# Wangkkkkkkkk/ORB-SLAM3

Measured on AMD Instinct MI355X. Metric: ORB extract+match frames/sec @752x480, 1000 feat, higher is better.
Workload: dtype u8; 1 GPU; configs[1]: 752x480 grayscale (synthetic, texture class 'dense', 16 distinct frames per rank), 1000 features, 8 levels, scale 1.2, FAST 20/7; batch of 1024 frames/GPU/step resident in HBM; extract + AssignFeaturesToGrid + SearchByProjection(frame, previous frame, th=15, mono; ORBmatcher.cc:2469-2711) of every frame, final match rows (claims, TH_HIGH, rotation-histogram cull) on the device; keypoin; launch=hipGraph replay (one hipGraphLaunch per step), keypoints_last_batch=1035840

## Files before the change

orb-slam3_amd/csrc/orbm_api.hip:

```cpp
#include "../../include/orbm.h"
#include "orbm_kernels.hip.h"

#include <cstdarg>
#include <cstdio>
#include <algorithm>
#include <chrono>
#include <climits>
#include <cmath>
#include <cstring>
#include <string>
#include <utility>
#include <vector>

using namespace orbmk;

#ifdef ORBX_AB
static inline const char* ab_env(const char* name) { return getenv(name); }
#else
static inline const char* ab_env(const char*) { return nullptr; }
#endif

static thread_local std::string g_merr;
static void set_merr(const char* fmt, ...) {
    char buf[512];
// ... 960 lines not shown
    int nFused = 0;
    for (int i = 0; i < nq; ++i) {
        best_idx[i] = -1;
        if (!valid[i] || cnt[i] == 0) continue;
        int bestDist = chi2_gate ? 256 : INT_MAX, bestIdx = -1;
        for (int c = 0; c < cnt[i]; ++c) {
            const int k = idx[(size_t)i * cap + c];
            if (chi2_gate) {
                const orbm_kp_t& kp = kf->kps[k];
                if (kf->uright && kf->uright[k] >= 0) {
                    const float ex = u[i] - kp.x, ey = v[i] - kp.y, er = ur[i] - kf->uright[k];
                    const float e2 = ex * ex + ey * ey + er * er;
                    if (e2 * inv_sigma2[kp.octave] > 7.8) continue;
                } else {
                    const float ex = u[i] - kp.x, ey = v[i] - kp.y;
                    const float e2 = ex * ex + ey * ey;
                    if (e2 * inv_sigma2[kp.octave] > 5.99) continue;
                }
            }
            const int d = dist[(size_t)i * cap + c];
            if (d < bestDist) { bestDist = d; bestIdx = k; }
        }
        if (bestDist <= ORBM_TH_LOW) { best_idx[i] = bestIdx; nFused++; }
    }
    return nFused;
}

static int sim3_one_way(orbm* m, const orbm_frame_t* src, const orbm_frame_t* dst, const float* sf_dst, const uint8_t* valid,
                        const float* u, const float* v, const int32_t* level, const uint8_t* qdesc, float th, std::vector<int>& vnMatch) {
    const int nq = src->n;
    vnMatch.assign(nq, -1);
    std::vector<float> qr(nq);
    std::vector<int> minl(nq), maxl(nq);
    for (int i = 0; i < nq; ++i) {
        if (!valid[i]) { qr[i] = -1.f; minl[i] = 0; maxl[i] = -1; continue; }
        qr[i] = th * sf_dst[level[i]]; minl[i] = level[i] - 1; maxl[i] = level[i];
    }
    int cap = std::max(1, std::min(dst->n, 2048));
    std::vector<int> cnt, idx, dist;
    orbm_frame_t f = *dst; f.uright = nullptr;
    int rc = window_pass(m, &f, nq, u, v, qr.data(), minl.data(), maxl.data(), nullptr, nullptr, qdesc, cap, cnt, idx, dist);
    if (rc) return rc;
    for (int i = 0; i < nq; ++i) {
        if (!valid[i]) continue;
        int bestDist = INT_MAX, bestIdx = -1;
        for (int c = 0; c < cnt[i]; ++c) {
            const int d = dist[(size_t)i * cap + c];
            if (d < bestDist) { bestDist = d; bestIdx = idx[(size_t)i * cap + c]; }
        }
        if (bestDist <= ORBM_TH_HIGH) vnMatch[i] = bestIdx;
    }
    return ORBM_OK;
}

int orbm_search_by_sim3(orbm_t* m, const orbm_frame_t* kf1, const orbm_frame_t* kf2, const float* sf1, const float* sf2,
                        const uint8_t* valid1, const float* u1, const float* v1, const int32_t* level1, const uint8_t* qdesc1,
                        const uint8_t* valid2, const float* u2, const float* v2, const int32_t* level2, const uint8_t* qdesc2,
                        float th, int32_t* matches12) {
    if (!m || !kf1 || !kf2) return ORBM_E_INVALID;
    std::vector<int> vnMatch1, vnMatch2;
    int rc = sim3_one_way(m, kf1, kf2, sf2, valid1, u1, v1, level1, qdesc1, th, vnMatch1);
    if (rc) return rc;
    rc = sim3_one_way(m, kf2, kf1, sf1, valid2, u2, v2, level2, qdesc2, th, vnMatch2);
    if (rc) return rc;
    int nFound = 0;
    for (int i1 = 0; i1 < kf1->n; ++i1) {
        matches12[i1] = -1;
        const int idx2 = vnMatch1[i1];
        if (idx2 >= 0 && vnMatch2[idx2] == i1) { matches12[i1] = idx2; nFound++; }
    }
    return nFound;
}

int orbm_grid_build_batch_async(orbm_t* m, const orbm_kp_t* kps, const int32_t* counts, int nframes, int cap,
                                float min_x, float min_y, float inv_w, float inv_h, int32_t* grid_start, int32_t* grid_idx) {
    if (!m || !kps || !counts || !grid_start || !grid_idx || nframes < 1 || cap < 1 || cap > 65535) return ORBM_E_INVALID;
    MHIPCHK(hipSetDevice(m->device));
    int n2 = 64; while (n2 < cap) n2 <<= 1;
    if ((size_t)n2 * 4 > 150 * 1024) { set_merr("too many keypoints per frame for the LDS sort"); return ORBM_E_CAPACITY; }
    if (cap > GRID_CS_MAX && n2 * 4 > 48 * 1024) MHIPCHK(hipFuncSetAttribute((const void*)k_grid_build_batch, hipFuncAttributeMaxDynamicSharedMemorySize, n2 * 4));
    MHIPCHK(rec_time(m, m->e2));
    m->gridFirst = true;
    if (cap <= GRID_CS_MAX)
        hipLaunchKernelGGL(k_grid_build_batch_cs, dim3(nframes), dim3(256), grid_cs_lds(cap), m->stream, (const KpIn*)kps, counts, cap,
                           min_x, min_y, inv_w, inv_h, grid_start, grid_idx);
    else
        hipLaunchKernelGGL(k_grid_build_batch, dim3(nframes), dim3(256), (size_t)n2 * 4, m->stream, (const KpIn*)kps, counts, cap, n2,
                           min_x, min_y, inv_w, inv_h, grid_start, grid_idx);
    MHIPCHK(hipGetLastError());
    return ORBM_OK;
}

static ScaleTab scale_tab(const float* sf, int nlevels) {
    ScaleTab st;
    for (int i = 0; i < 12; ++i) st.sf[i] = i < nlevels ? sf[i] : sf[nlevels - 1];
    return st;
}

static int lp_capacity(const char* call, int cap, int q_stride, int nlevels, int nbatch, const char* batch_name) {
    if (cap > 65535) { set_merr("%s: %d keypoint slots per frame (the candidate words hold 65535)", call, cap); return ORBM_E_CAPACITY; }
    if (q_stride > ORBM_LP_MAX_QUERIES) { set_merr("%s: q_stride %d above %d", call, q_stride, (int)ORBM_LP_MAX_QUERIES); return ORBM_E_CAPACITY; }
    if (nlevels > 12) { set_merr("%s: %d scale levels (the scale table holds 12)", call, nlevels); return ORBM_E_CAPACITY; }
    if (nbatch > 65535) { set_merr("%s: %d %s in one call (at most 65535)", call, nbatch, batch_name); return ORBM_E_CAPACITY; }
    return ORBM_OK;
}

int orbm_track_window_batch_async(orbm_t* m, const orbm_kp_t* kps, const uint8_t* desc, const int32_t* counts, int cap,
                                  const int32_t* grid_start, const int32_t* grid_idx,
                                  float min_x, float min_y, float inv_w, float inv_h,
                                  int q_first, int t_first, int npairs, float th, const float* sf, int nlevels,
                                  float dx, float dy, int32_t* best_idx, int32_t* best_dist, int32_t* second_dist) {
    if (!m || !kps || !desc || !counts || !grid_start || !grid_idx || !best_idx || !best_dist || !second_dist || npairs < 1 ||
        nlevels < 1 || nlevels > 12 || !sf) return ORBM_E_INVALID;
    MHIPCHK(hipSetDevice(m->device));
    const ScaleTab st = scale_tab(sf, nlevels);
    MHIPCHK(rec_time(m, m->e0));
    hipLaunchKernelGGL(k_track_window, dim3((cap + 3) / 4, npairs), dim3(256), 0, m->stream, (const KpIn*)kps, desc, counts, cap,
                       grid_start, grid_idx, min_x, min_y, inv_w, inv_h, q_first, t_first, th, st, dx, dy, best_idx, best_dist, second_dist);
    MHIPCHK(rec_time(m, m->e1));
    MHIPCHK(hipGetLastError());
    m->timed = true;
    return ORBM_OK;
}

int orbm_search_by_projection_batch_async(orbm_t* m, const orbm_kp_t* kps, const uint8_t* desc, const int32_t* counts, int cap,
                                          const int32_t* grid_start, const int32_t* grid_idx,
                                          float min_x, float min_y, float inv_w, float inv_h,
                                          int q_first, int t_first, int npairs, float th, const float* sf, int nlevels,
                                          float dx, float dy, const uint8_t* t_blocked, const uint8_t* q_obs, int check_orientation,
                                          int32_t* match, int32_t* nmatches) {
    if (!m || !kps || !desc || !counts || !grid_start || !grid_idx || !match || !nmatches || npairs < 1 || cap < 1 || cap > 65535 ||
        nlevels < 1 || nlevels > 12 || !sf || q_first < 0 || t_first < 0) return ORBM_E_INVALID;
    MHIPCHK(hipSetDevice(m->device));
    const ScaleTab st = scale_tab(sf, nlevels);
    const size_t lds = (size_t)(2 * ((cap + 31) >> 5) + 32 + cap) * sizeof(unsigned);
    if (lds > 64 * 1024) { set_merr("SearchByProjection batch: %d keypoint slots per frame need %zu B of LDS (limit 64 KB, ~16 000 slots)", cap, lds); return ORBM_E_INVALID; }
    const size_t rows = (size_t)npairs * cap;
    const size_t bCnt = (rows * sizeof(int) + 255) & ~(size_t)255, bKeys = (rows * TK_K * sizeof(unsigned) + 255) & ~(size_t)255,
                 bAcc = (rows * sizeof(unsigned) + 255) & ~(size_t)255, bEnt = rows * sizeof(uint4);
    uint8_t* scr = batch_scratch(m, bCnt + bKeys + bAcc + bEnt);
    if (!scr) { set_merr("SearchByProjection batch scratch of %zu B unavailable (inside a capture, run the call once eagerly first)", bCnt + bKeys + bAcc + bEnt); return ORBM_E_HIP; }
    int* topCnt = (int*)scr; unsigned* topKeys = (unsigned*)(scr + bCnt); unsigned* acc = (unsigned*)(scr + bCnt + bKeys);
    uint4* ent = (uint4*)(scr + bCnt + bKeys + bAcc);
    const float factor = ORBM_HISTO_LENGTH / 360.0f;
    MHIPCHK(rec_time(m, m->e0));
#ifdef ORBX_AB
    if (ab_env("ORBM_TOPK_WAVE"))
        hipLaunchKernelGGL(k_track_topk, dim3((cap + 3) / 4, npairs), dim3(256), 0, m->stream, (const KpIn*)kps, desc, counts, cap,
                           grid_start, grid_idx, min_x, min_y, inv_w, inv_h, q_first, t_first, th, st, dx, dy, factor, topCnt, topKeys);
    else
#endif
    {
        hipLaunchKernelGGL(k_track_pack, dim3((cap + 255) / 256, npairs), dim3(256), 0, m->stream, (const KpIn*)kps, cap, grid_start, grid_idx, t_first, ent);
        hipLaunchKernelGGL(k_track_topk16, dim3((cap + 15) / 16, npairs), dim3(256), 0, m->stream, (const KpIn*)kps, desc, counts, cap,
                           grid_start, ent, min_x, min_y, inv_w, inv_h, q_first, t_first, th, st, dx, dy, factor, topCnt, topKeys);
    }
#ifdef ORBX_AB
    if (ab_env("ORBM_CLAIM_V1"))
        hipLaunchKernelGGL(k_track_claim, dim3(npairs), dim3(64), lds, m->stream, (const KpIn*)kps, desc, counts, cap,
                           grid_start, grid_idx, min_x, min_y, inv_w, inv_h, q_first, t_first, th, st, dx, dy, factor, topCnt, topKeys,
                           t_blocked, q_obs, check_orientation, acc, match, nmatches);
    else
#endif
    hipLaunchKernelGGL(k_track_claim64, dim3(npairs), dim3(64), lds, m->stream, (const KpIn*)kps, desc, counts, cap,
                       grid_start, grid_idx, min_x, min_y, inv_w, inv_h, q_first, t_first, th, st, dx, dy, factor, topCnt, topKeys,
                       t_blocked, q_obs, check_orientation, acc, match, nmatches);
    MHIPCHK(rec_time(m, m->e1));
    MHIPCHK(hipGetLastError());
    m->timed = true;
    return ORBM_OK;
}

int orbm_search_by_projection_points_batch_async(orbm_t* m, const orbm_kp_t* kps, const uint8_t* desc, const int32_t* counts, int cap,
                                                 const int32_t* grid_start, const int32_t* grid_idx,
                                                 float min_x, float min_y, float inv_w, float inv_h, int t_first, int nframes,
                                                 const float* uright, const uint8_t* t_blocked, const int32_t* nq, int q_stride,
                                                 const uint8_t* in_view, const float* proj_x, const float* proj_y, const float* proj_xr,
                                                 const float* view_cos, const int32_t* level, const float* depth, float th_far,
                                                 const uint8_t* qdesc, const uint8_t* mp_obs, int q_shared,
                                                 float th, float nnratio, const float* scale_factors_host, int nlevels,
                                                 int32_t* match, int32_t* nmatches) {
    if (!m || !kps || !desc || !counts || !grid_start || !grid_idx || !nq || !in_view || !proj_x || !proj_y || !view_cos || !level ||
        !qdesc || !mp_obs || !match || !nmatches || !scale_factors_host || (uright && !proj_xr)) {
        set_merr("SearchByProjection points batch: a required array is NULL (proj_xr is required with uright)");
        return ORBM_E_INVALID;
    }
    if (nframes < 1 || cap < 1 || q_stride < 1 || t_first < 0 || nlevels < 1) {
        set_merr("SearchByProjection points batch: nframes, cap, q_stride and nlevels must be >= 1, t_first >= 0");
        return ORBM_E_INVALID;
    }
    if (const int rc = lp_capacity("SearchByProjection points batch", cap, q_stride, nlevels, nframes, "frames")) return rc;
    MHIPCHK(hipSetDevice(m->device));
    const ScaleTab st = scale_tab(scale_factors_host, nlevels);
    const size_t lds = (size_t)(((cap + 31) >> 5) + 32 + 64 * TK_K) * sizeof(unsigned);
    const size_t rows = (size_t)nframes * q_stride;
    const size_t bCnt = (rows * sizeof(int) + 255) & ~(size_t)255, bKeys = rows * TK_K * sizeof(unsigned), bR = rows * sizeof(float);
    uint8_t* scr = batch_scratch(m, bCnt + bKeys + bR);
    if (!scr) { set_merr("SearchByProjection points batch scratch of %zu B unavailable (inside a capture, run the call once eagerly first)", bCnt + bKeys + bR); return ORBM_E_HIP; }
    int* topCnt = (int*)scr; unsigned* topKeys = (unsigned*)(scr + bCnt); float* topR = (float*)(scr + bCnt + bKeys);
    LpRows R;
    R.nq = nq; R.q_stride = q_stride;
    R.in_view = in_view; R.px = proj_x; R.py = proj_y; R.pxr = proj_xr; R.view_cos = view_cos; R.level = level;
    R.depth = depth; R.th_far = th_far;
    R.qdesc = qdesc; R.mp_obs = mp_obs; R.q_shared = q_shared != 0;
    R.th = th; R.nlevels = nlevels;
    MHIPCHK(rec_time(m, m->e0));
    hipLaunchKernelGGL(k_lp_topk, dim3((q_stride + 3) / 4, nframes), dim3(256), 0, m->stream, (const KpIn*)kps, desc, cap, grid_start, grid_idx,
                       min_x, min_y, inv_w, inv_h, t_first, uright, R, st, topCnt, topKeys, topR);
    hipLaunchKernelGGL(k_lp_claim, dim3(nframes), dim3(64), lds, m->stream, (const KpIn*)kps, desc, counts, cap, grid_start, grid_idx,
                       min_x, min_y, inv_w, inv_h, t_first, uright, t_blocked, R, nnratio, topCnt, topKeys, topR, match, nmatches);
    MHIPCHK(rec_time(m, m->e1));
    MHIPCHK(hipGetLastError());
    m->timed = true;
    return ORBM_OK;
}

int orbm_search_by_projection_frame_batch_async(orbm_t* m, const orbm_kp_t* kps, const uint8_t* desc, const int32_t* counts, int cap,
                                                const int32_t* grid_start, const int32_t* grid_idx,
                                                float min_x, float min_y, float inv_w, float inv_h, int t_first, int npairs,
                                                const float* uright, float mbf, const uint8_t* t_blocked, const uint8_t* dir,
                                                const int32_t* nq, int q_stride, const uint8_t* valid, const float* u, const float* v,
                                                const float* invzc, const int32_t* octave, const float* angle, const uint8_t* qdesc,
                                                const uint8_t* mp_obs, float th, int retry_below, const float* scale_factors_host, int nlevels,
                                                int check_orientation, int32_t* match, int32_t* nmatches, uint8_t* retried) {
    if (!m || !kps || !desc || !counts || !grid_start || !grid_idx || !nq || !valid || !u || !v || !octave || !angle || !qdesc || !mp_obs ||
        !match || !nmatches || !scale_factors_host || (uright && !invzc)) {
        set_merr("SearchByProjection frame batch: a required array is NULL (invzc is required with uright)");
        return ORBM_E_INVALID;
    }
    if (npairs < 1 || cap < 1 || q_stride < 1 || t_first < 0 || nlevels < 1 || retry_below < 0) {
        set_merr("SearchByProjection frame batch: npairs, cap, q_stride and nlevels must be >= 1, t_first and retry_below >= 0");
        return ORBM_E_INVALID;
    }
    if (const int rc = lp_capacity("SearchByProjection frame batch", cap, q_stride, nlevels, npairs, "pairs")) return rc;
    MHIPCHK(hipSetDevice(m->device));
    const ScaleTab st = scale_tab(scale_factors_host, nlevels);
    const size_t lds = (size_t)(((cap + 31) >> 5) + 32 + 64 * TK_K) * sizeof(unsigned);
    const size_t rows = (size_t)npairs * q_stride;
    const size_t bCnt = (rows * sizeof(int) + 255) & ~(size_t)255, bKeys = rows * TK_K * sizeof(unsigned), bAcc = rows * sizeof(unsigned),
                 bR = rows * sizeof(float);
    uint8_t* scr = batch_scratch(m, bCnt + bKeys + bAcc + bR);
    if (!scr) { set_merr("SearchByProjection frame batch scratch of %zu B unavailable (inside a capture, run the call once eagerly first)", bCnt + bKeys + bAcc + bR); return ORBM_E_HIP; }
    int* topCnt = (int*)scr; unsigned* topKeys = (unsigned*)(scr + bCnt); unsigned* acc = (unsigned*)(scr + bCnt + bKeys);
    float* topR = (float*)(scr + bCnt + bKeys + bAcc);
    MmRows R;
    R.nq = nq; R.q_stride = q_stride;
    R.valid = valid; R.u = u; R.v = v; R.invzc = invzc; R.octave = octave; R.angle = angle;
    R.qdesc = qdesc; R.mp_obs = mp_obs; R.dir = dir;
    R.mbf = mbf; R.factor = ORBM_HISTO_LENGTH / 360.0f;
    R.nlevels = nlevels; R.retry_below = retry_below; R.check_ori = check_orientation != 0;
    const dim3 gTop((q_stride + 3) / 4, npairs);
    MHIPCHK(rec_time(m, m->e0));
    hipLaunchKernelGGL(k_mm_topk<false>, gTop, dim3(256), 0, m->stream, (const KpIn*)kps, desc, cap, grid_start, grid_idx,
                       min_x, min_y, inv_w, inv_h, t_first, uright, R, st, th, nmatches, topCnt, topKeys, topR);
    hipLaunchKernelGGL(k_mm_claim<false>, dim3(npairs), dim3(64), lds, m->stream, (const KpIn*)kps, desc, counts, cap, grid_start, grid_idx,
                       min_x, min_y, inv_w, inv_h, t_first, uright, t_blocked, R, topCnt, topKeys, topR, acc, match, nmatches, retried);
    if (retry_below > 0) {
        const float th2 = 2 * th;
        hipLaunchKernelGGL(k_mm_topk<true>, gTop, dim3(256), 0, m->stream, (const KpIn*)kps, desc, cap, grid_start, grid_idx,
                           min_x, min_y, inv_w, inv_h, t_first, uright, R, st, th2, nmatches, topCnt, topKeys, topR);
        hipLaunchKernelGGL(k_mm_claim<true>, dim3(npairs), dim3(64), lds, m->stream, (const KpIn*)kps, desc, counts, cap, grid_start, grid_idx,
                           min_x, min_y, inv_w, inv_h, t_first, uright, nullptr, R, topCnt, topKeys, topR, acc, match, nmatches, retried);
    }
    MHIPCHK(rec_time(m, m->e1));
    MHIPCHK(hipGetLastError());
    m->timed = true;
    return ORBM_OK;
}

int orbm_project_last_frame_batch_async(orbm_t* m, int npairs, const float* tcw_cur, const float* tcw_last, const int32_t* nq, int q_stride,
                                        const float* x3dw, const uint8_t* has_mp, const float* k_host, const float* bounds_host, float mb, int mono,
                                        uint8_t* valid, float* u, float* v, float* invzc, uint8_t* dir) {
    if (!m || !tcw_cur || !tcw_last || !nq || !x3dw || !has_mp || !k_host || !bounds_host || !valid || !u || !v || !invzc || !dir) {
        set_merr("project last frame batch: a required array is NULL");
        return ORBM_E_INVALID;
    }
    if (npairs < 1 || q_stride < 1) { set_merr("project last frame batch: npairs and q_stride must be >= 1"); return ORBM_E_INVALID; }
    if (q_stride > ORBM_LP_MAX_QUERIES) { set_merr("project last frame batch: q_stride %d above %d", q_stride, (int)ORBM_LP_MAX_QUERIES); return ORBM_E_CAPACITY; }
    if (npairs > 65535) { set_merr("project last frame batch: %d pairs in one call (at most 65535)", npairs); return ORBM_E_CAPACITY; }
    MHIPCHK(hipSetDevice(m->device));
    MmProj P;
    for (int i = 0; i < 4; ++i) { P.k[i] = k_host[i]; P.bounds[i] = bounds_host[i]; }
    P.mb = mb; P.mono = mono != 0; P.q_stride = q_stride;
    hipLaunchKernelGGL(k_mm_project, dim3((q_stride + 255) / 256, npairs), dim3(256), 0, m->stream, tcw_cur, tcw_last, nq, x3dw, has_mp, P,
                       valid, u, v, invzc, dir);
    MHIPCHK(hipGetLastError());
    return ORBM_OK;
}

int orbm_fuse_batch_async(orbm_t* m, int npairs,
                          int nkf_rows, int cap, const orbm_kp_t* kps_kf, const uint8_t* desc_kf, const float* uright_kf,
                          const int32_t* grid_start, const int32_t* grid_idx, float min_x, float min_y, float inv_w, float inv_h,
                          const int32_t* kf_row, const float* tcw, const float* ow,
                          const int32_t* nq, int q_stride, const uint8_t* valid,
                          const float* pw, const float* normal, const float* min_dist, const float* max_dist, const uint8_t* qdesc, int q_shared,
                          const float* k_host, const float* bounds_host, float bf,
                          float th, int chi2_gate, const float* scale_factors_host, const float* inv_sigma2_host,
                          float log_scale_factor, int nlevels,
                          int32_t* best_idx, int32_t* nfused, int32_t* level_out) {
    if (!m || !kps_kf || !desc_kf || !grid_start || !grid_idx || !tcw || !ow || !nq || !valid || !pw || !normal || !min_dist || !max_dist ||
        !qdesc || !k_host || !bounds_host || !scale_factors_host || (chi2_gate && !inv_sigma2_host) || !best_idx || !nfused) {
        set_merr("Fuse batch: a required array is NULL (inv_sigma2 is required with chi2_gate)");
        return ORBM_E_INVALID;
    }
    if (npairs < 1 || nkf_rows < 1 || cap < 1 || q_stride < 1 || nlevels < 1 || !std::isfinite(th)) {
        set_merr("Fuse batch: npairs, nkf_rows, cap, q_stride and nlevels must be >= 1, th finite");
// ... 913 lines not shown
```

orb-slam3_amd/csrc/orbm_kernels.hip.h:

```cpp
#pragma once
#include <hip/hip_runtime.h>
#include <stdint.h>

namespace orbmk {

typedef unsigned long long u64;

__device__ __forceinline__ int ham256(const u64 a[4], u64 b0, u64 b1, u64 b2, u64 b3) {
    return __popcll(a[0] ^ b0) + __popcll(a[1] ^ b1) + __popcll(a[2] ^ b2) + __popcll(a[3] ^ b3);
}

__device__ __forceinline__ unsigned bcnt_acc(unsigned x, unsigned acc) {
#if __HIP_DEVICE_COMPILE__
    unsigned r;
    asm("v_bcnt_u32_b32 %0, %1, %2" : "=v"(r) : "v"(x), "v"(acc));
    return r;
#else
    return (unsigned)__builtin_popcount(x) + acc;
#endif
}

__device__ __forceinline__ unsigned umed3(unsigned a, unsigned b, unsigned c) {
#if __HIP_DEVICE_COMPILE__
    unsigned r;
// ... 1106 lines not shown
        if (sz > max1) { max3 = max2; max2 = max1; max1 = sz; i3 = i2; i2 = i1; i1 = i; }
        else if (sz > max2) { max3 = max2; max2 = sz; i3 = i2; i2 = i; }
        else if (sz > max3) { max3 = sz; i3 = i; }
    }
    if ((float)max2 < 0.1f * (float)max1) { i2 = -1; i3 = -1; }
    else if ((float)max3 < 0.1f * (float)max1) i3 = -1;
    return Max3{i1, i2, i3};
}

__device__ __forceinline__ int rot_cull(const unsigned int* hist, const unsigned int* acc, int nacc, int* mrow, int lane) {
    const Max3 m3 = three_maxima(hist);
    const int i1 = m3.i1, i2 = m3.i2, i3 = m3.i3;
    int pruned = 0;
    for (int e = lane; e < nacc; e += 64) {
        const unsigned int v = acc[e];
        const int bin = (int)(v >> 16), k = (int)(v & 0xFFFFu);
        if (bin != i1 && bin != i2 && bin != i3) { mrow[k] = -2; ++pruned; }
    }
#pragma unroll
    for (int o = 32; o > 0; o >>= 1) pruned += __shfl_xor(pruned, o);
    return pruned;
}

__device__ __forceinline__ void put_topk(int* out_cnt, float* out_r, unsigned int* out_keys, size_t o, int cnt, float r, const u64 (&top)[TK_K]) {
    out_cnt[o] = cnt;
    out_r[o] = r;
    uint4* ok = (uint4*)(out_keys + o * TK_K);
    ok[0] = make_uint4(cand_word(top[0]), cand_word(top[1]), cand_word(top[2]), cand_word(top[3]));
    ok[1] = make_uint4(cand_word(top[4]), cand_word(top[5]), cand_word(top[6]), cand_word(top[7]));
}

#ifdef ORBX_AB
__global__ __launch_bounds__(256) void k_track_topk(const KpIn* __restrict__ kps, const uint8_t* __restrict__ desc,
                                                    const int* __restrict__ counts, int cap, const int* __restrict__ grid_start,
                                                    const int* __restrict__ grid_idx, float min_x, float min_y, float inv_w, float inv_h,
                                                    int q_first, int t_first, float th, ScaleTab st, float dx, float dy, float factor,
                                                    int* __restrict__ out_cnt, unsigned int* __restrict__ out_keys) {
    const int lane = threadIdx.x & 63;
    const int pair = blockIdx.y;
    const int qf = q_first + pair, tf = t_first + pair;
    const int q = blockIdx.x * 4 + (threadIdx.x >> 6);
    if (q >= min(counts[qf], cap)) return;
    const KpIn kq = kps[(size_t)qf * cap + q];
    const KpIn* kt = kps + (size_t)tf * cap;
    const uint8_t* dt = desc + (size_t)tf * cap * 32;
    const int* gs = grid_start + (size_t)tf * (64 * 48 + 1);
    const int* gi = grid_idx + (size_t)tf * cap;
    const float x = kq.x + dx, y = kq.y + dy, r = th * st.sf[kq.octave];
    const int minLevel = kq.octave - 1, maxLevel = kq.octave + 1;
    const unsigned INV = 0xFFFFFFFFu;
    unsigned topKey[TK_K], topPay[TK_K];
#pragma unroll
    for (int i = 0; i < TK_K; ++i) { topKey[i] = INV; topPay[i] = INV; }
    int cnt = 0;
    const int nMinCellX = max(0, (int)floorf((x - min_x - r) * inv_w));
    const int nMaxCellX = min(63, (int)ceilf((x - min_x + r) * inv_w));
    const int nMinCellY = max(0, (int)floorf((y - min_y - r) * inv_h));
    const int nMaxCellY = min(47, (int)ceilf((y - min_y + r) * inv_h));
    if (nMinCellX < 64 && nMaxCellX >= 0 && nMinCellY < 48 && nMaxCellY >= 0) {
        const uint4* qp = (const uint4*)(desc + ((size_t)qf * cap + q) * 32);
        const uint4 qlo = qp[0], qhi = qp[1];
        const u64 a[4] = {(u64)qlo.x | ((u64)qlo.y << 32), (u64)qlo.z | ((u64)qlo.w << 32),
                          (u64)qhi.x | ((u64)qhi.y << 32), (u64)qhi.z | ((u64)qhi.w << 32)};
        const unsigned long long lt = (1ull << lane) - 1ull;
        const int ncols = nMaxCellX - nMinCellX + 1;
        int cj0 = 0, clen = 0;
        if (lane < ncols) {
            const int ix = nMinCellX + lane;
            cj0 = gs[ix * 48 + nMinCellY];
            clen = gs[ix * 48 + nMaxCellY + 1] - cj0;
        }
        int total;
        const int coff = wave_excl_scan(clen, &total);
        bool first = true;
        for (int base = 0; base < total; base += 64) {
            const int t = base + lane;
            int myj0 = 0, myoff = 0;
            for (int c = 0; c < ncols; ++c) {
                const int oc = __builtin_amdgcn_readlane(coff, c), jc = __builtin_amdgcn_readlane(cj0, c);
                if (t >= oc) { myoff = oc; myj0 = jc; }
            }
            bool ok = false;
            int k = 0;
            float ang = 0.f;
            if (t < total) {
                k = gi[myj0 + (t - myoff)];
                const KpIn kp = kt[k];
                ok = !(kp.octave < minLevel) && !(kp.octave > maxLevel);
                if (!(fabsf(kp.x - x) < r && fabsf(kp.y - y) < r)) ok = false;
                ang = kp.angle;
            }
            const unsigned long long bal = __ballot(ok);
            if (bal == 0) continue;
            unsigned key = INV, pay = INV;
            if (ok) {
                const int pos = cnt + __popcll(bal & lt);
                const uint4* tp = (const uint4*)(dt + (size_t)k * 32);
                const uint4 lo = tp[0], hi = tp[1];
                const int d = ham256(a, (u64)lo.x | ((u64)lo.y << 32), (u64)lo.z | ((u64)lo.w << 32),
                                     (u64)hi.x | ((u64)hi.y << 32), (u64)hi.z | ((u64)hi.w << 32));
                float rot = kq.angle - ang;
                if (rot < 0.0f) rot += 360.0f;
                int bin = (int)roundf(rot * factor);
                if (bin == 30) bin = 0;
                if (bin < 0 || bin >= 30) bin = TK_NOBIN;
                key = ((unsigned)d << 16) | (unsigned)pos;
                pay = ((unsigned)bin << 16) | (unsigned)k;
            }
            cnt += __popcll(bal);
            if (first) {
#pragma unroll
                for (int i = 0; i < TK_K; ++i) {
                    const unsigned m = wave_min_u32(key);
                    if (m == INV) break;
                    const int src = __ffsll((long long)__ballot(key == m)) - 1;
                    topKey[i] = m; topPay[i] = (unsigned)__builtin_amdgcn_readlane((int)pay, src);
                    if (lane == src) key = INV;
                }
                first = false;
            } else {
                for (int rnd = 0; rnd < TK_K; ++rnd) {
                    const unsigned m = wave_min_u32(key);
                    if (m >= topKey[TK_K - 1]) break;
                    const int src = __ffsll((long long)__ballot(key == m)) - 1;
                    unsigned ck = m, cp = (unsigned)__builtin_amdgcn_readlane((int)pay, src);
                    if (lane == src) key = INV;
#pragma unroll
                    for (int i = 0; i < TK_K; ++i) {
                        const bool sw = ck < topKey[i];
                        const unsigned tk = topKey[i], tp2 = topPay[i];
                        topKey[i] = sw ? ck : tk; topPay[i] = sw ? cp : tp2;
                        ck = sw ? tk : ck; cp = sw ? tp2 : cp;
                    }
                }
            }
        }
    }
    if (lane == 0) {
        const size_t o = (size_t)pair * cap + q;
        out_cnt[o] = cnt;
#pragma unroll
        for (int i = 0; i < TK_K; ++i)
            out_keys[o * TK_K + i] = topKey[i] == INV ? 0xFFFFFFFFu : ((topKey[i] >> 16) << 21) | (topPay[i] & 0x1FFFFFu);
    }
}

#endif

struct Tk16 {
    const uint4* ent; const uint8_t* dt; int cap;
    float x, y, r, qangle, factor; int minLevel, maxLevel;
    int total, ncols, qr, l16, wr;
};
template <int NJ, bool FB>
__device__ __forceinline__ void tk16_pass(const Tk16& c, const u64 (&a)[4], int base, int& cnt, const int2 (*sCol)[64], const int (*sAdj)[64], uint2 (*sK)[16], uint2 (*sTop)[TK_K]) {
    const unsigned INV = 0xFFFFFFFFu;
    int t[NJ], eidx[NJ];
    const int cnt0 = cnt;
#pragma unroll
    for (int j = 0; j < NJ; ++j) t[j] = base + 16 * j + c.l16;
    if (!FB) {
#pragma unroll
        for (int j = 0; j < NJ; ++j) eidx[j] = t[j] < c.total ? t[j] + sAdj[c.qr][t[j]] : 0;
    } else {
        int off[NJ], j0[NJ];
#pragma unroll
        for (int j = 0; j < NJ; ++j) { off[j] = 0; j0[j] = 0; }
        for (int col = 0; __any(col < c.ncols); ++col) {
            const int2 e = sCol[c.qr][col];
            const bool in = col < c.ncols;
#pragma unroll
            for (int j = 0; j < NJ; ++j) if (in && t[j] >= e.x) { off[j] = e.x; j0[j] = e.y; }
        }
#pragma unroll
        for (int j = 0; j < NJ; ++j) eidx[j] = t[j] < c.total ? j0[j] + (t[j] - off[j]) : 0;
    }
    int k[NJ];
    float kx[NJ], ky[NJ], ang[NJ];
    int oct[NJ];
#pragma unroll
    for (int j = 0; j < NJ; ++j) {
        const uint4 e = c.ent[eidx[j]];
        kx[j] = __uint_as_float(e.x); ky[j] = __uint_as_float(e.y); ang[j] = __uint_as_float(e.z);
        oct[j] = (int)(e.w >> 16); k[j] = (int)(e.w & 0xFFFFu);
    }
    bool ok[NJ];
    uint4 lo[NJ], hi[NJ];
#pragma unroll
    for (int j = 0; j < NJ; ++j) {
        ok[j] = t[j] < c.total && !(oct[j] < c.minLevel) && !(oct[j] > c.maxLevel) && (fabsf(kx[j] - c.x) < c.r && fabsf(ky[j] - c.y) < c.r);
        const uint4* tp = (const uint4*)(c.dt + (size_t)(ok[j] ? k[j] : 0) * 32);
        lo[j] = tp[0]; hi[j] = tp[1];
    }
    const unsigned below = (1u << c.l16) - 1u;
    unsigned key[NJ + 1], word[NJ + 1];
    int posj[NJ];
#pragma unroll
    for (int j = 0; j < NJ; ++j) {
        const unsigned rowbits = (unsigned)(__ballot(ok[j]) >> (16 * c.wr)) & 0xFFFFu;
        const int pos = cnt + __popc(rowbits & below);
        posj[j] = pos;
        const int d = ham256(a, (u64)lo[j].x | ((u64)lo[j].y << 32), (u64)lo[j].z | ((u64)lo[j].w << 32),
                             (u64)hi[j].x | ((u64)hi[j].y << 32), (u64)hi[j].z | ((u64)hi[j].w << 32));
        float rot = c.qangle - ang[j];
        if (rot < 0.0f) rot += 360.0f;
        int bin = (int)roundf(rot * c.factor);
        if (bin == 30) bin = 0;
        if (bin < 0 || bin >= 30) bin = TK_NOBIN;
        key[j] = ok[j] ? ((unsigned)d << 16) | (unsigned)pos : INV;
        word[j] = ((unsigned)d << 21) | ((unsigned)bin << 16) | (unsigned)k[j];
        cnt += __popc(rowbits);
    }
    key[NJ] = INV; word[NJ] = INV;
    if (FB && c.l16 < TK_K) { const uint2 pv = sTop[c.qr][c.l16]; key[NJ] = pv.x; word[NJ] = pv.y; }
    const int nv = cnt - cnt0;
    if (!FB && (NJ == 1 || !__any(nv > 16))) {
        unsigned k1 = key[0], w1 = word[0];
        if (NJ > 1) {
#pragma unroll
            for (int j = 0; j < NJ; ++j) if (key[j] != INV) sK[c.qr][posj[j] - cnt0] = make_uint2(key[j], word[j]);
            __builtin_amdgcn_fence(__ATOMIC_RELEASE, "wavefront");
            __builtin_amdgcn_wave_barrier();
            const uint2 e = sK[c.qr][c.l16];
            k1 = c.l16 < nv ? e.x : INV; w1 = e.y;
        }
        int rank = 0;
        unsigned rk = k1;
#pragma unroll
        for (int i = 0; i < 15; ++i) {
            rk = (unsigned)__builtin_amdgcn_update_dpp((int)rk, (int)rk, 0x121, 0xf, 0xf, false);
            rank += rk < k1 ? 1 : 0;
        }
        if (k1 != INV && rank < TK_K) sTop[c.qr][rank] = make_uint2(k1, w1);
    } else {
#pragma unroll
        for (int i = 0; i < TK_K; ++i) {
            unsigned mine = key[0];
#pragma unroll
            for (int j = 1; j <= (FB ? NJ : NJ - 1); ++j) mine = min(mine, key[j]);
            const unsigned m = row16_min_u32(mine);
            if (!__any(m != INV)) break;
            if (mine == m && m != INV) {
                unsigned w = word[0];
#pragma unroll
                for (int j = 1; j <= (FB ? NJ : NJ - 1); ++j) if (key[j] == m) w = word[j];
                sTop[c.qr][i] = make_uint2(m, w);
#pragma unroll
                for (int j = 0; j <= (FB ? NJ : NJ - 1); ++j) if (key[j] == m) key[j] = INV;
            }
        }
    }
    __builtin_amdgcn_fence(__ATOMIC_RELEASE, "wavefront");
    __builtin_amdgcn_wave_barrier();
}

__global__ __launch_bounds__(256) void k_track_pack(const KpIn* __restrict__ kps, int cap, const int* __restrict__ grid_start,
                                                    const int* __restrict__ grid_idx, int t_first, uint4* __restrict__ ent) {
    const int pair = blockIdx.y, tf = t_first + pair;
    const int pos = blockIdx.x * 256 + threadIdx.x;
    const int n = min(grid_start[(size_t)tf * (64 * 48 + 1) + 64 * 48], cap);
    if (pos >= n) return;
    const int k = grid_idx[(size_t)tf * cap + pos];
    const KpIn kp = kps[(size_t)tf * cap + k];
    ent[(size_t)pair * cap + pos] = make_uint4(__float_as_uint(kp.x), __float_as_uint(kp.y), __float_as_uint(kp.angle), ((unsigned)kp.octave << 16) | (unsigned)k);
}

__global__ __launch_bounds__(256) void k_track_topk16(const KpIn* __restrict__ kps, const uint8_t* __restrict__ desc,
                                                      const int* __restrict__ counts, int cap, const int* __restrict__ grid_start,
                                                      const uint4* __restrict__ ent, float min_x, float min_y, float inv_w, float inv_h,
                                                      int q_first, int t_first, float th, ScaleTab st, float dx, float dy, float factor,
                                                      int* __restrict__ out_cnt, unsigned int* __restrict__ out_keys) {
    __shared__ int2 sCol[16][64];
    __shared__ uint2 sTop[16][TK_K];
    __shared__ int sAdj[16][64];
    __shared__ uint2 sK[16][16];
    const int lane = threadIdx.x & 63, l16 = threadIdx.x & 15, wr = lane >> 4, qr = threadIdx.x >> 4;
    const int pair = blockIdx.y;
    const int qf = q_first + pair, tf = t_first + pair;
    const int nq = min(counts[qf], cap);
    if ((int)blockIdx.x * 16 >= nq) return;
    const int q = blockIdx.x * 16 + qr;
    const bool live = q < nq;
    const KpIn kq = kps[(size_t)qf * cap + (live ? q : 0)];
    const int* gs = grid_start + (size_t)tf * (64 * 48 + 1);
    const float x = kq.x + dx, y = kq.y + dy, r = th * st.sf[kq.octave];
    const unsigned INV = 0xFFFFFFFFu;
    const int nMinCellX = max(0, (int)floorf((x - min_x - r) * inv_w));
    const int nMaxCellX = min(63, (int)ceilf((x - min_x + r) * inv_w));
    const int nMinCellY = max(0, (int)floorf((y - min_y - r) * inv_h));
    const int nMaxCellY = min(47, (int)ceilf((y - min_y + r) * inv_h));
    const bool hit = live && nMinCellX < 64 && nMaxCellX >= 0 && nMinCellY < 48 && nMaxCellY >= 0;
    const int ncols = hit ? nMaxCellX - nMinCellX + 1 : 0;
    u64 a[4];
    load_desc(desc + ((size_t)qf * cap + (live ? q : 0)) * 32, a);
    if (l16 < TK_K) sTop[qr][l16] = make_uint2(INV, INV);
    int total = 0;
    for (int cb = 0; __any(cb < ncols); cb += 16) {
        const int c = cb + l16;
        int cj0 = 0, clen = 0;
        if (c < ncols) {
            const int ix = nMinCellX + c;
            cj0 = gs[ix * 48 + nMinCellY];
            clen = gs[ix * 48 + nMaxCellY + 1] - cj0;
        }
        int sc = clen;
        sc += __builtin_amdgcn_update_dpp(0, sc, 0x111, 0xf, 0xf, true);
        sc += __builtin_amdgcn_update_dpp(0, sc, 0x112, 0xf, 0xf, true);
        sc += __builtin_amdgcn_update_dpp(0, sc, 0x114, 0xf, 0xf, true);
        sc += __builtin_amdgcn_update_dpp(0, sc, 0x118, 0xf, 0xf, true);
        const int excl = total + sc - clen;
        if (c < ncols) sCol[qr][c] = make_int2(excl, cj0);
        for (int e = 0; __any(e < clen && excl + e < 64); ++e)
            if (e < clen && excl + e < 64) sAdj[qr][excl + e] = cj0 - excl;
        const int s0 = __builtin_amdgcn_readlane(sc, 15), s1 = __builtin_amdgcn_readlane(sc, 31),
                  s2 = __builtin_amdgcn_readlane(sc, 47), s3 = __builtin_amdgcn_readlane(sc, 63);
        total += wr == 0 ? s0 : wr == 1 ? s1 : wr == 2 ? s2 : s3;
    }
    __builtin_amdgcn_fence(__ATOMIC_RELEASE, "wavefront");
    __builtin_amdgcn_wave_barrier();
    Tk16 c;
    c.ent = ent + (size_t)pair * cap; c.dt = desc + (size_t)tf * cap * 32; c.cap = cap;
    c.x = x; c.y = y; c.r = r; c.qangle = kq.angle; c.factor = factor; c.minLevel = kq.octave - 1; c.maxLevel = kq.octave + 1;
    c.total = total; c.ncols = ncols; c.qr = qr; c.l16 = l16; c.wr = wr;
    const int maxTotal = max(max(__builtin_amdgcn_readlane(total, 0), __builtin_amdgcn_readlane(total, 16)),
                             max(__builtin_amdgcn_readlane(total, 32), __builtin_amdgcn_readlane(total, 48)));
    int cnt = 0;
    for (int base = 0; base < maxTotal; base += 64) {
        const int nj = min(4, (maxTotal - base + 15) >> 4);
        if (base == 0) {
            if (nj == 1) tk16_pass<1, false>(c, a, base, cnt, sCol, sAdj, sK, sTop);
            else if (nj == 2) tk16_pass<2, false>(c, a, base, cnt, sCol, sAdj, sK, sTop);
            else if (nj == 3) tk16_pass<3, false>(c, a, base, cnt, sCol, sAdj, sK, sTop);
            else tk16_pass<4, false>(c, a, base, cnt, sCol, sAdj, sK, sTop);
        } else {
            if (nj <= 2) tk16_pass<2, true>(c, a, base, cnt, sCol, sAdj, sK, sTop);
            else tk16_pass<4, true>(c, a, base, cnt, sCol, sAdj, sK, sTop);
        }
    }
    if (live) {
        const size_t o = (size_t)pair * cap + q;
        if (l16 == 0) out_cnt[o] = cnt;
        if (l16 < TK_K) { const uint2 e = sTop[qr][l16]; out_keys[o * TK_K + l16] = e.x == INV ? INV : e.y; }
    }
}

#ifdef ORBX_AB
__global__ __launch_bounds__(64) void k_track_claim(const KpIn* __restrict__ kps, const uint8_t* __restrict__ desc,
                                                    const int* __restrict__ counts, int cap, const int* __restrict__ grid_start,
                                                    const int* __restrict__ grid_idx, float min_x, float min_y, float inv_w, float inv_h,
                                                    int q_first, int t_first, float th, ScaleTab st, float dx, float dy, float factor,
                                                    const int* __restrict__ topCnt, const unsigned int* __restrict__ topKeys,
                                                    const uint8_t* __restrict__ t_blocked, const uint8_t* __restrict__ q_obs, int check_ori,
                                                    unsigned int* __restrict__ accepted, int* __restrict__ match, int* __restrict__ nmatches) {
    extern __shared__ unsigned int tk_lds[];
    const int lane = threadIdx.x, pair = blockIdx.x;
    const int qf = q_first + pair, tf = t_first + pair;
    const int nq = min(counts[qf], cap), nt = min(counts[tf], cap);
    const int nwords = (cap + 31) >> 5;
    unsigned int* blk = tk_lds;
    unsigned int* hist = tk_lds + nwords;
    unsigned int* obsb = hist + 32;
    int* mrow = match + (size_t)pair * cap;
    unsigned int* acc = accepted + (size_t)pair * cap;
    const uint8_t* tb = t_blocked ? t_blocked + (size_t)tf * cap : nullptr;
    const uint8_t* qo = q_obs ? q_obs + (size_t)qf * cap : nullptr;
    for (int w = lane; w < nwords; w += 64) { blk[w] = bits_word(tb, nt, w, 0u); obsb[w] = bits_word(qo, nq, w, 0xFFFFFFFFu); }
    if (lane < 32) hist[lane] = 0;
    for (int k = lane; k < cap; k += 64) mrow[k] = -1;
    __syncthreads();
    const size_t rowBase = (size_t)pair * cap;
    const int sub = lane >> 3;
    int nm = 0, nacc = 0;
    const int qLast = max(nq - 1, 0);
    unsigned int ak0, ak1, ak2, ak3;
    int ac0, ac1, ac2, ac3;
    auto fetch = [&](int qi, unsigned int& k_, int& c_) {
        const int qc = min(qi, qLast);
        k_ = topKeys[(rowBase + qc) * TK_K + (lane & 7)];
        c_ = topCnt[rowBase + qc];
    };
    fetch(sub, ak0, ac0); fetch(8 + sub, ak1, ac1); fetch(16 + sub, ak2, ac2); fetch(24 + sub, ak3, ac3);
    for (int G = 0; G < nq; G += 32) {
      unsigned int bk0, bk1, bk2, bk3;
      int bc0, bc1, bc2, bc3;
      fetch(G + 32 + sub, bk0, bc0); fetch(G + 40 + sub, bk1, bc1); fetch(G + 48 + sub, bk2, bc2); fetch(G + 56 + sub, bk3, bc3);
#pragma clang loop unroll(disable)
      for (int s4 = 0; s4 < 4; ++s4) {
        const int g0 = G + 8 * s4;
        if (g0 >= nq) break;
        const bool ql = g0 + sub < nq;
        const unsigned int kraw = s4 == 0 ? ak0 : s4 == 1 ? ak1 : s4 == 2 ? ak2 : ak3;
        const int craw = s4 == 0 ? ac0 : s4 == 1 ? ac1 : s4 == 2 ? ac2 : ac3;
        const unsigned int key = ql ? kraw : 0xFFFFFFFFu;
        const int cnt = ql ? craw : 0;
        const int qme = min(g0 + sub, qLast);
        const unsigned ob = (obsb[qme >> 5] >> (qme & 31)) & 1u;
        const unsigned long long obsMask = __ballot(ob != 0);
        const bool valid = key != 0xFFFFFFFFu;
        const unsigned int myk = key & 0xFFFFu;
        bool blocked = valid && ((blk[myk >> 5] >> (myk & 31)) & 1u);
        const int gend = min(8, nq - g0);
        {
            const unsigned long long fr = __ballot(valid && !blocked);
            const unsigned m8 = (unsigned)(fr >> (8 * sub)) & 0xFFu;
            const unsigned pick = (unsigned)__shfl((int)key, (sub << 3) + (m8 ? __ffs((int)m8) - 1 : 0));
            const bool qlive = g0 + sub < nq;
            const bool take = qlive && m8 != 0 && (pick >> 21) <= 100u;
            const unsigned pk = pick & 0xFFFFu;
            bool clash = qlive && m8 == 0 && cnt > TK_K;
#pragma unroll
            for (int e = 0; e < 7; ++e) {
                const unsigned ke = (unsigned)__builtin_amdgcn_readlane((int)pk, 8 * e);
                const int te = __builtin_amdgcn_readlane((int)take, 8 * e);
                if (te && take && sub > e && ke == pk) clash = true;
            }
            if (!__any(clash)) {
                const bool lead = (lane & 7) == 0 && take;
                const unsigned bin = (pick >> 16) & 31u;
                const bool withBin = lead && check_ori && bin != TK_NOBIN;
                const unsigned long long tb = __ballot(lead), bb = __ballot(withBin);
                if (lead) {
                    mrow[pk] = g0 + sub;
                    if (ob != 0) atomicOr(&blk[pk >> 5], 1u << (pk & 31));
                }
                if (withBin) {
                    acc[nacc + __popcll(bb & ((1ull << lane) - 1ull))] = pk | (bin << 16);
                    atomicAdd(&hist[bin], 1u);
                }
                nm += __popcll(tb);
                nacc += __popcll(bb);
                continue;
            }
        }
        for (int s = 0; s < gend; ++s) {
            const int qi = g0 + s;
            const unsigned long long sel = 0xFFull << (8 * s);
            const unsigned long long bal = __ballot(valid && !blocked) & sel;
            unsigned int best = 0xFFFFFFFFu;
            if (bal) best = (unsigned int)__builtin_amdgcn_readlane((int)key, __ffsll((long long)bal) - 1);
            else {
                const int c = __builtin_amdgcn_readlane(cnt, 8 * s);
                if (c > TK_K) {
                    const KpIn kq = kps[(size_t)qf * cap + qi];
                    const Win w = {kq.x + dx, kq.y + dy, th * st.sf[kq.octave], 0.f, kq.octave - 1, kq.octave + 1};
                    u64 a[4], top[TK_K];
                    load_desc(desc + ((size_t)qf * cap + qi) * 32, a);
                    int c2;
                    win_sweep<false>(w, RotBinPay{kq.angle, factor}, kps + (size_t)tf * cap, desc + (size_t)tf * cap * 32, nullptr,
                                     grid_start + (size_t)tf * (64 * 48 + 1), grid_idx + (size_t)tf * cap, min_x, min_y, inv_w, inv_h, a, blk, lane, c2, top);
                    best = cand_word(top[0]);
                }
            }
            if (best == 0xFFFFFFFFu) continue;
            const int d = (int)(best >> 21);
            if (d > 100) continue;
            const unsigned int k = best & 0xFFFFu, bin = (best >> 16) & 31u;
            const bool obs = (obsMask >> (8 * s)) & 1ull;
            if (obs && valid && myk == k) blocked = true;
            if (lane == 0) {
                mrow[k] = qi;
                if (obs) atomicOr(&blk[k >> 5], 1u << (k & 31));
                if (check_ori && bin != TK_NOBIN) { acc[nacc] = k | (bin << 16); atomicAdd(&hist[bin], 1u); }
            }
            ++nm;
            if (check_ori && bin != TK_NOBIN) ++nacc;
        }
      }
      ak0 = bk0; ak1 = bk1; ak2 = bk2; ak3 = bk3; ac0 = bc0; ac1 = bc1; ac2 = bc2; ac3 = bc3;
    }
    __syncthreads();
    if (check_ori) nm -= rot_cull(hist, acc, nacc, mrow, lane);
    if (lane == 0) nmatches[pair] = nm;
}

#endif

__global__ __launch_bounds__(64) void k_track_claim64(const KpIn* __restrict__ kps, const uint8_t* __restrict__ desc,
                                                    const int* __restrict__ counts, int cap, const int* __restrict__ grid_start,
                                                    const int* __restrict__ grid_idx, float min_x, float min_y, float inv_w, float inv_h,
                                                    int q_first, int t_first, float th, ScaleTab st, float dx, float dy, float factor,
                                                    const int* __restrict__ topCnt, const unsigned int* __restrict__ topKeys,
                                                    const uint8_t* __restrict__ t_blocked, const uint8_t* __restrict__ q_obs, int check_ori,
                                                    unsigned int* __restrict__ accepted, int* __restrict__ match, int* __restrict__ nmatches) {
    extern __shared__ unsigned int tk_lds[];
    const int lane = threadIdx.x, pair = blockIdx.x;
    const int qf = q_first + pair, tf = t_first + pair;
    const int nq = min(counts[qf], cap), nt = min(counts[tf], cap);
    const int nwords = (cap + 31) >> 5;
    unsigned int* blk = tk_lds;
    unsigned int* hist = tk_lds + nwords;
    unsigned int* obsb = hist + 32;
    unsigned int* tag = obsb + nwords;
    int* mrow = match + (size_t)pair * cap;
    unsigned int* acc = accepted + (size_t)pair * cap;
    const uint8_t* tb = t_blocked ? t_blocked + (size_t)tf * cap : nullptr;
    const uint8_t* qo = q_obs ? q_obs + (size_t)qf * cap : nullptr;
    for (int w = lane; w < nwords; w += 64) { blk[w] = bits_word(tb, nt, w, 0u); obsb[w] = bits_word(qo, nq, w, 0xFFFFFFFFu); }
// ... 1230 lines not shown
```

Baseline: 304,100 frames/s.

## Filter candidates before fetching descriptors in topk16 pass, compact survivors via LDS

The default top-k pass now reads only the packed entry (position, angle, octave) for each candidate, applies the level and radius tests first, and compacts the survivors into 16-wide rows through LDS. Descriptors are then loaded and Hamming distances computed only for those survivors. The first pass ranks its keys with a DPP rank instead of an iterative min extraction, and later passes merge against the current top list. The old fetch-everything path stays behind an A/B flag; the change cuts descriptor loads and popcount work at the cost of extra LDS round-trips and wave barriers.

```diff
diff --git a/orb-slam3_amd/csrc/orbm_api.hip b/orb-slam3_amd/csrc/orbm_api.hip
--- a/orb-slam3_amd/csrc/orbm_api.hip
+++ b/orb-slam3_amd/csrc/orbm_api.hip
@@ -1136,6 +1136,12 @@
 #endif
     {
         hipLaunchKernelGGL(k_track_pack, dim3((cap + 255) / 256, npairs), dim3(256), 0, m->stream, (const KpIn*)kps, cap, grid_start, grid_idx, t_first, ent);
+#ifdef ORBX_AB
+        if (ab_env("ORBM_TOPK16_V1"))
+            hipLaunchKernelGGL(k_track_topk16_v1, dim3((cap + 15) / 16, npairs), dim3(256), 0, m->stream, (const KpIn*)kps, desc, counts, cap,
+                               grid_start, ent, min_x, min_y, inv_w, inv_h, q_first, t_first, th, st, dx, dy, factor, topCnt, topKeys);
+        else
+#endif
         hipLaunchKernelGGL(k_track_topk16, dim3((cap + 15) / 16, npairs), dim3(256), 0, m->stream, (const KpIn*)kps, desc, counts, cap,
                            grid_start, ent, min_x, min_y, inv_w, inv_h, q_first, t_first, th, st, dx, dy, factor, topCnt, topKeys);
     }
diff --git a/orb-slam3_amd/csrc/orbm_kernels.hip.h b/orb-slam3_amd/csrc/orbm_kernels.hip.h
--- a/orb-slam3_amd/csrc/orbm_kernels.hip.h
+++ b/orb-slam3_amd/csrc/orbm_kernels.hip.h
@@ -1282,8 +1282,124 @@
     float x, y, r, qangle, factor; int minLevel, maxLevel;
     int total, ncols, qr, l16, wr;
 };
+__device__ __forceinline__ void tk16_cand(const Tk16& c, const u64 (&a)[4], const uint4& lo, const uint4& hi, float ang, int k, int pos, bool ok,
+                                          unsigned& key, unsigned& word) {
+    const int d = ham256(a, (u64)lo.x | ((u64)lo.y << 32), (u64)lo.z | ((u64)lo.w << 32), (u64)hi.x | ((u64)hi.y << 32), (u64)hi.z | ((u64)hi.w << 32));
+    float rot = c.qangle - ang;
+    if (rot < 0.0f) rot += 360.0f;
+    int bin = (int)roundf(rot * c.factor);
+    if (bin == 30) bin = 0;
+    if (bin < 0 || bin >= 30) bin = TK_NOBIN;
+    key = ok ? ((unsigned)d << 16) | (unsigned)pos : 0xFFFFFFFFu;
+    word = ((unsigned)d << 21) | ((unsigned)bin << 16) | (unsigned)k;
+}
+
+__device__ __forceinline__ void tk16_merge(const Tk16& c, unsigned k1, unsigned w1, unsigned pk, unsigned pw, uint2 (*sTop)[TK_K]) {
+    const unsigned INV = 0xFFFFFFFFu;
+#pragma unroll
+    for (int i = 0; i < TK_K; ++i) {
+        const unsigned mine = min(k1, pk);
+        const unsigned m = row16_min_u32(mine);
+        if (!__any(m != INV)) break;
+        if (mine == m && m != INV) {
+            sTop[c.qr][i] = make_uint2(m, pk == m ? pw : w1);
+            if (pk == m) pk = INV; else k1 = INV;
+        }
+    }
+}
+
 template <int NJ, bool FB>
 __device__ __forceinline__ void tk16_pass(const Tk16& c, const u64 (&a)[4], int base, int& cnt, const int2 (*sCol)[64], const int (*sAdj)[64], uint2 (*sK)[16], uint2 (*sTop)[TK_K]) {
+    const unsigned INV = 0xFFFFFFFFu;
+    int t[NJ], eidx[NJ];
+    const int cnt0 = cnt;
+#pragma unroll
+    for (int j = 0; j < NJ; ++j) t[j] = base + 16 * j + c.l16;
+    if (!FB) {
+#pragma unroll
+        for (int j = 0; j < NJ; ++j) eidx[j] = t[j] < c.total ? t[j] + sAdj[c.qr][t[j]] : 0;
+    } else {
+        int off[NJ], j0[NJ];
+#pragma unroll
+        for (int j = 0; j < NJ; ++j) { off[j] = 0; j0[j] = 0; }
+        for (int col = 0; __any(col < c.ncols); ++col) {
+            const int2 e = sCol[c.qr][col];
+            const bool in = col < c.ncols;
+#pragma unroll
+            for (int j = 0; j < NJ; ++j) if (in && t[j] >= e.x) { off[j] = e.x; j0[j] = e.y; }
+        }
+#pragma unroll
+        for (int j = 0; j < NJ; ++j) eidx[j] = t[j] < c.total ? j0[j] + (t[j] - off[j]) : 0;
+    }
+    int k[NJ];
+    float kx[NJ], ky[NJ], ang[NJ];
+    int oct[NJ];
+#pragma unroll
+    for (int j = 0; j < NJ; ++j) {
+        const uint4 e = c.ent[eidx[j]];
+        kx[j] = __uint_as_float(e.x); ky[j] = __uint_as_float(e.y); ang[j] = __uint_as_float(e.z);
+        oct[j] = (int)(e.w >> 16); k[j] = (int)(e.w & 0xFFFFu);
+    }
+    const unsigned below = (1u << c.l16) - 1u;
+    bool ok[NJ];
+    int posj[NJ];
+#pragma unroll
+    for (int j = 0; j < NJ; ++j) {
+        ok[j] = t[j] < c.total && !(oct[j] < c.minLevel) && !(oct[j] > c.maxLevel) && (fabsf(kx[j] - c.x) < c.r && fabsf(ky[j] - c.y) < c.r);
+        const unsigned rowbits = (unsigned)(__ballot(ok[j]) >> (16 * c.wr)) & 0xFFFFu;
+        posj[j] = cnt + __popc(rowbits & below);
+        cnt += __popc(rowbits);
+    }
+    const int nv = cnt - cnt0;
+#pragma unroll
+    for (int r = 0; r < NJ; ++r) {
+        if (r > 0 && !__any(nv > 16 * r)) break;
+        bool ok1 = ok[0];
+        int k1 = k[0], pos1 = posj[0];
+        float ang1 = ang[0];
+        if (NJ > 1) {
+#pragma unroll
+            for (int j = 0; j < NJ; ++j) {
+                const int rel = posj[j] - cnt0 - 16 * r;
+                if (ok[j] && (unsigned)rel < 16u) sK[c.qr][rel] = make_uint2(((unsigned)posj[j] << 16) | (unsigned)k[j], __float_as_uint(ang[j]));
+            }
+            __builtin_amdgcn_fence(__ATOMIC_RELEASE, "wavefront");
+            __builtin_amdgcn_wave_barrier();
+            const uint2 e = sK[c.qr][c.l16];
+            ok1 = 16 * r + c.l16 < nv; k1 = (int)(e.x & 0xFFFFu); pos1 = (int)(e.x >> 16); ang1 = __uint_as_float(e.y);
+        }
+        const uint4* tp = (const uint4*)(c.dt + (size_t)(ok1 ? k1 : 0) * 32);
+        const uint4 lo = tp[0], hi = tp[1];
+        unsigned key, word;
+        tk16_cand(c, a, lo, hi, ang1, k1, pos1, ok1, key, word);
+        if (!FB && r == 0) {
+            int rank = 0;
+            unsigned rk = key;
+#pragma unroll
+            for (int i = 0; i < 15; ++i) {
+                rk = (unsigned)__builtin_amdgcn_update_dpp((int)rk, (int)rk, 0x121, 0xf, 0xf, false);
+                rank += rk < key ? 1 : 0;
+            }
+            if (key != INV && rank < TK_K) sTop[c.qr][rank] = make_uint2(key, word);
+        } else {
+            unsigned pk = INV, pw = INV;
+            if (c.l16 < TK_K) { const uint2 pv = sTop[c.qr][c.l16]; pk = pv.x; pw = pv.y; }
+            tk16_merge(c, key, word, pk, pw, sTop);
+        }
+        __builtin_amdgcn_fence(__ATOMIC_RELEASE, "wavefront");
+        __builtin_amdgcn_wave_barrier();
+    }
+}
+struct Tk16Filter {
+    template <int NJ, bool FB>
+    static __device__ __forceinline__ void run(const Tk16& c, const u64 (&a)[4], int base, int& cnt, const int2 (*sCol)[64], const int (*sAdj)[64], uint2 (*sK)[16], uint2 (*sTop)[TK_K]) {
+        tk16_pass<NJ, FB>(c, a, base, cnt, sCol, sAdj, sK, sTop);
+    }
+};
+
+#ifdef ORBX_AB
+template <int NJ, bool FB>
+__device__ __forceinline__ void tk16_pass_v1(const Tk16& c, const u64 (&a)[4], int base, int& cnt, const int2 (*sCol)[64], const int (*sAdj)[64], uint2 (*sK)[16], uint2 (*sTop)[TK_K]) {
     const unsigned INV = 0xFFFFFFFFu;
     int t[NJ], eidx[NJ];
     const int cnt0 = cnt;
@@ -1383,6 +1499,13 @@
     __builtin_amdgcn_fence(__ATOMIC_RELEASE, "wavefront");
     __builtin_amdgcn_wave_barrier();
 }
+struct Tk16FetchAll {
+    template <int NJ, bool FB>
+    static __device__ __forceinline__ void run(const Tk16& c, const u64 (&a)[4], int base, int& cnt, const int2 (*sCol)[64], const int (*sAdj)[64], uint2 (*sK)[16], uint2 (*sTop)[TK_K]) {
+        tk16_pass_v1<NJ, FB>(c, a, base, cnt, sCol, sAdj, sK, sTop);
+    }
+};
+#endif
 
 __global__ __launch_bounds__(256) void k_track_pack(const KpIn* __restrict__ kps, int cap, const int* __restrict__ grid_start,
                                                     const int* __restrict__ grid_idx, int t_first, uint4* __restrict__ ent) {
@@ -1395,11 +1518,12 @@
     ent[(size_t)pair * cap + pos] = make_uint4(__float_as_uint(kp.x), __float_as_uint(kp.y), __float_as_uint(kp.angle), ((unsigned)kp.octave << 16) | (unsigned)k);
 }
 
-__global__ __launch_bounds__(256) void k_track_topk16(const KpIn* __restrict__ kps, const uint8_t* __restrict__ desc,
-                                                      const int* __restrict__ counts, int cap, const int* __restrict__ grid_start,
-                                                      const uint4* __restrict__ ent, float min_x, float min_y, float inv_w, float inv_h,
-                                                      int q_first, int t_first, float th, ScaleTab st, float dx, float dy, float factor,
-                                                      int* __restrict__ out_cnt, unsigned int* __restrict__ out_keys) {
+template <class Pass>
+__device__ __forceinline__ void tk16_body(const KpIn* __restrict__ kps, const uint8_t* __restrict__ desc,
+                                          const int* __restrict__ counts, int cap, const int* __restrict__ grid_start,
+                                          const uint4* __restrict__ ent, float min_x, float min_y, float inv_w, float inv_h,
+                                          int q_first, int t_first, float th, const ScaleTab& st, float dx, float dy, float factor,
+                                          int* __restrict__ out_cnt, unsigned int* __restrict__ out_keys) {
     __shared__ int2 sCol[16][64];
     __shared__ uint2 sTop[16][TK_K];
     __shared__ int sAdj[16][64];
@@ -1458,13 +1582,13 @@
     for (int base = 0; base < maxTotal; base += 64) {
         const int nj = min(4, (maxTotal - base + 15) >> 4);
         if (base == 0) {
-            if (nj == 1) tk16_pass<1, false>(c, a, base, cnt, sCol, sAdj, sK, sTop);
-            else if (nj == 2) tk16_pass<2, false>(c, a, base, cnt, sCol, sAdj, sK, sTop);
-            else if (nj == 3) tk16_pass<3, false>(c, a, base, cnt, sCol, sAdj, sK, sTop);
-            else tk16_pass<4, false>(c, a, base, cnt, sCol, sAdj, sK, sTop);
+            if (nj == 1) Pass::template run<1, false>(c, a, base, cnt, sCol, sAdj, sK, sTop);
+            else if (nj == 2) Pass::template run<2, false>(c, a, base, cnt, sCol, sAdj, sK, sTop);
+            else if (nj == 3) Pass::template run<3, false>(c, a, base, cnt, sCol, sAdj, sK, sTop);
+            else Pass::template run<4, false>(c, a, base, cnt, sCol, sAdj, sK, sTop);
         } else {
-            if (nj <= 2) tk16_pass<2, true>(c, a, base, cnt, sCol, sAdj, sK, sTop);
-            else tk16_pass<4, true>(c, a, base, cnt, sCol, sAdj, sK, sTop);
+            if (nj <= 2) Pass::template run<2, true>(c, a, base, cnt, sCol, sAdj, sK, sTop);
+            else Pass::template run<4, true>(c, a, base, cnt, sCol, sAdj, sK, sTop);
         }
     }
     if (live) {
@@ -1473,6 +1597,18 @@
         if (l16 < TK_K) { const uint2 e = sTop[qr][l16]; out_keys[o * TK_K + l16] = e.x == INV ? INV : e.y; }
     }
 }
+
+#define TK16_PARAMS const KpIn* __restrict__ kps, const uint8_t* __restrict__ desc, const int* __restrict__ counts, int cap,                 \
+                    const int* __restrict__ grid_start, const uint4* __restrict__ ent, float min_x, float min_y, float inv_w, float inv_h,    \
+                    int q_first, int t_first, float th, ScaleTab st, float dx, float dy, float factor, int* __restrict__ out_cnt,             \
+                    unsigned int* __restrict__ out_keys
+#define TK16_ARGS kps, desc, counts, cap, grid_start, ent, min_x, min_y, inv_w, inv_h, q_first, t_first, th, st, dx, dy, factor, out_cnt, out_keys
+__global__ __launch_bounds__(256) void k_track_topk16(TK16_PARAMS) { tk16_body<Tk16Filter>(TK16_ARGS); }
+#ifdef ORBX_AB
+__global__ __launch_bounds__(256) void k_track_topk16_v1(TK16_PARAMS) { tk16_body<Tk16FetchAll>(TK16_ARGS); }
+#endif
+#undef TK16_PARAMS
+#undef TK16_ARGS
 
 #ifdef ORBX_AB
 __global__ __launch_bounds__(64) void k_track_claim(const KpIn* __restrict__ kps, const uint8_t* __restrict__ desc,
```

Measured after the change: 311,800 frames/s (median of 6 runs). +2.5%, better.
